# CloudEngineHub/FairyGen

Measured on AMD Instinct MI355X. Metric: decoded frames/sec (sec/clip in config), Wan2.2-TI2V-5B 704x1280x121 @ 5 steps, higher is better.
Workload: dtype bf16

## Files before the change

### fairygen_amd/csrc/attention.hip

```cpp
#include "common.h"
#include <math.h>
#include <queue>
#include <type_traits>
#include <vector>

#include "attn_w4_asm.inc"
#include "attn_w4p_asm.inc"
#ifndef FG_ATTN_W4
#define FG_ATTN_W4 1
#endif

namespace {

constexpr int kD = 128;
constexpr int kBN = 64;
constexpr int kTileBytes = kBN * kD * 2;
constexpr float kDeferLog2 = 6.0f;

typedef __attribute__((address_space(3))) s16x4 lds_s16x4;

__device__ __forceinline__ int k_lds_off(int row, int chunk) { return row * 256 + ((chunk ^ (row & 15)) << 4); }
__device__ __forceinline__ int v_lds_off(int row, int chunk) {
    return 2048 * (row >> 3) + 512 * (chunk >> 2) + 64 * (row & 7) + 16 * ((chunk & 3) ^ ((row >> 2) & 3));
}
// ... 531 lines not shown
    std::priority_queue<double, std::vector<double>, std::greater<double>> free_at;
    for (int i = 0; i < cus; ++i) free_at.push((double)(full + (i < rem ? 1 : 0)));
    double last = (double)(full + (rem ? 1 : 0));
    for (int64_t i = 0; i < n_pieces; ++i) {
        const double t = free_at.top() + piece_cost;
        free_at.pop();
        free_at.push(t);
        last = t > last ? t : last;
    }
    return last;
}

static SplitChoice choose_split_uncached(int B, int64_t Nq, int64_t Nkv, int H, int cus, int64_t ws_limit) {
    const int64_t nqb = (Nq + kBM - 1) / kBM, bh = (int64_t)B * H;
    const int nt = (int)((Nkv + kBN - 1) / kBN);
    const int64_t per_piece = (int64_t)kBM * kD * 4 + (int64_t)kBM * 2 * 4;
    SplitChoice best{0, 1, 0, simulate_makespan(bh * nqb, 0, 0.0, cus)};
    const double base = best.makespan;
    const int s_list[] = {2, 3, 4, 5, 6, 8, 12, 16};
    for (int mode = 0; mode < 2; ++mode) {
        const int64_t R = mode == 0 ? 1 : nqb;
        if (mode == 0 && nqb < 2) continue;
        if (mode == 1 && bh * nqb > 4 * (int64_t)cus) continue;
        for (int S : s_list) {
            if (S * 8 > nt) break;
            const int64_t pieces = bh * R * S;
            const int64_t ws = pieces * per_piece;
            if (ws > ws_limit) continue;
            const double cost = 1.0 / S + 3.0 / nt + 0.004;
            const double ms = simulate_makespan(bh * (nqb - R), pieces, cost, cus);
            if (ms < best.makespan) best = SplitChoice{(int)R, S, ws, ms};
        }
    }
    if (best.makespan > 0.98 * base) best = SplitChoice{0, 1, 0, base};
    return best;
}

static SplitChoice choose_split(int B, int64_t Nq, int64_t Nkv, int H, int cus, int64_t ws_limit) {
    struct Key { int B, H, cus; int64_t Nq, Nkv, ws; SplitChoice val; };
    static thread_local Key memo[8];
    static thread_local int next = 0, filled = 0;
    for (int i = 0; i < filled; ++i) {
        const Key& e = memo[i];
        if (e.B == B && e.H == H && e.cus == cus && e.Nq == Nq && e.Nkv == Nkv && e.ws == ws_limit) return e.val;
    }
    const SplitChoice val = choose_split_uncached(B, Nq, Nkv, H, cus, ws_limit);
    memo[next] = Key{B, H, cus, Nq, Nkv, ws_limit, val};
    next = (next + 1) % 8;
    if (filled < 8) ++filled;
    return val;
}

static int device_cus() {
    static thread_local int cached_dev = -1, cached_cus = 256;
    int dev = 0;
    if (hipGetDevice(&dev) != hipSuccess) return 256;
    if (dev != cached_dev) {
        int n = 0;
        if (hipDeviceGetAttribute(&n, hipDeviceAttributeMultiprocessorCount, dev) == hipSuccess && n > 0) cached_cus = n;
        cached_dev = dev;
    }
    return cached_cus * (256 / kBM);
}

}

extern "C" int64_t fg_attn_workspace_bytes(int B, int64_t Nq, int64_t Nkv, int H) {
    if (B <= 0 || Nq <= 0 || Nkv <= 0 || H <= 0) return 0;
    return choose_split(B, Nq, Nkv, H, device_cus(), (int64_t)1 << 40).ws_bytes;
}

extern "C" int fg_attn_split_choice(int B, int64_t Nq, int64_t Nkv, int H, int64_t workspace_bytes, int* R, int* S) {
    FG_CHECK_ARG(B > 0 && Nq > 0 && Nkv > 0 && H > 0 && R && S, "fg_attn_split_choice: bad arguments");
    const SplitChoice sc = choose_split(B, Nq, Nkv, H, device_cus(), workspace_bytes);
    *R = sc.R;
    *S = sc.S;
    return FG_OK;
}

extern "C" int fg_attn_fwd_bf16(const void* q, int64_t ldq, const void* k, int64_t ldk, const void* v, int64_t ldv,
                                void* out, int B, int64_t Nq, int64_t Nkv, int H, int D, float scale, void* workspace,
                                int64_t workspace_bytes, fg_stream_t stream) {
    FG_CHECK_ARG(q && k && v && out, "fg_attn_fwd_bf16: null pointer");
    FG_CHECK_ARG(D == kD, "fg_attn_fwd_bf16: only head_dim 128 is supported (got %d)", D);
    FG_CHECK_ARG(B > 0 && H > 0 && Nq > 0 && Nkv > 0, "fg_attn_fwd_bf16: B, H, Nq, Nkv must be positive");
    FG_CHECK_ARG(scale > 0.f, "fg_attn_fwd_bf16: scale must be positive");
    const int64_t hd = (int64_t)H * D;
    FG_CHECK_ARG(ldq >= hd && ldk >= hd && ldv >= hd && ldq % 8 == 0 && ldk % 8 == 0 && ldv % 8 == 0,
                 "fg_attn_fwd_bf16: leading dimensions must be >= H*D and multiples of 8");
    FG_CHECK_ARG(FG_ALIGNED16(q) && FG_ALIGNED16(k) && FG_ALIGNED16(v) && FG_ALIGNED16(out) && FG_ALIGNED16(workspace),
                 "fg_attn_fwd_bf16: pointers must be 16-byte aligned");
    FG_CHECK_ARG(workspace_bytes >= 0 && (workspace != nullptr || workspace_bytes == 0), "fg_attn_fwd_bf16: bad workspace");
    const int64_t nqb = (Nq + kBM - 1) / kBM;
    FG_CHECK_ARG((Nkv + 6 * kBN) * ldk * 2 < (1ll << 32) && (Nkv + 6 * kBN) * ldv * 2 < (1ll << 32),
                 "fg_attn_fwd_bf16: K/V of one batch element must span < 4 GiB (32-bit buffer offsets)");
    FG_CHECK_ARG(Nq * ldq * 2 < (1ll << 32) && Nq * hd * 2 < (1ll << 32),
                 "fg_attn_fwd_bf16: Q / O of one batch element must span < 4 GiB (32-bit buffer offsets)");
    const SplitChoice sc = choose_split(B, Nq, Nkv, H, device_cus(), workspace_bytes);
    AttnParams P;
    P.q = (const bf16*)q; P.k = (const bf16*)k; P.v = (const bf16*)v; P.out = (bf16*)out;
    P.ldq = ldq; P.ldk = ldk; P.ldv = ldv; P.Nq = Nq; P.Nkv = Nkv; P.H = H;
    P.nqb = (int)nqb; P.R = sc.R; P.S = sc.S; P.nfull = (int)(nqb - sc.R);
    const int64_t total_direct = (int64_t)B * H * P.nfull, pieces = (int64_t)B * H * sc.R * sc.S;
    FG_CHECK_ARG(total_direct + pieces < (1ll << 30), "fg_attn_fwd_bf16: grid too large");
    P.total_direct = (int)total_direct;
    P.scale_log2e = scale * 1.4426950408889634f;
    P.o_part = (float*)workspace;
    P.ml_part = (float*)workspace + pieces * kBM * kD;
#if FG_ATTN_VARIANT == 4
    hipLaunchKernelGGL((attn_fwd_kernel<4, 1>), dim3((unsigned)(total_direct + pieces)), dim3(256), 0, (hipStream_t)stream, P);
#else
#if FG_ATTN_W4
    static const bool use_w4 = [] { const char* e = getenv("FAIRYGEN_ATTN_W4"); return e ? atoi(e) != 0 : true; }();
    if (Nkv > 1024 && use_w4) {
        static const hipError_t attr0 = hipFuncSetAttribute(reinterpret_cast<const void*>(attn_fwd_w4_kernel<false>),
// ... 27 lines not shown
```

### fairygen_amd/csrc/common.h

```cpp
#pragma once
#include <hip/hip_runtime.h>
#include <stdint.h>
#include <stdio.h>
#include "../../include/fairygen_hip.h"

typedef __bf16 bf16;
typedef __attribute__((ext_vector_type(8))) __bf16 bf16x8;
typedef __attribute__((ext_vector_type(4))) __bf16 bf16x4;
typedef __attribute__((ext_vector_type(2))) __bf16 bf16x2;
typedef __attribute__((ext_vector_type(16))) float f32x16;
typedef __attribute__((ext_vector_type(4))) float f32x4;
typedef __attribute__((ext_vector_type(4))) short s16x4;
typedef __attribute__((ext_vector_type(4))) uint32_t u32x4;
typedef __attribute__((ext_vector_type(2))) uint32_t u32x2;

#define FG_WAVE 64

void fg_set_error(const char* fmt, ...);

#define FG_CHECK_ARG(cond, ...)                                  \
    do {                                                         \
        if (!(cond)) {                                           \
            fg_set_error(__VA_ARGS__);                           \
            return FG_EINVAL;                                    \
        }                                                        \
    } while (0)

#define FG_ALIGNED16(p) ((((uintptr_t)(p)) & 15) == 0)

static inline int fg_launch_status(const char* what) {
    hipError_t e = hipGetLastError();
    if (e != hipSuccess) {
        fg_set_error("%s: launch failed: %s", what, hipGetErrorString(e));
        return FG_ELAUNCH;
    }
    return FG_OK;
}

__device__ __forceinline__ float rbf(float x) { return (float)(bf16)x; }

__device__ __forceinline__ float silu_f(float x) { return x / (1.0f + __expf(-x)); }
__device__ __forceinline__ float gelu_tanh_f(float x) {
    const float kBeta = 0.7978845608028654f, kKappa = 0.044715f;
    const float u = kBeta * (x + kKappa * x * x * x);
    const float e = __expf(2.0f * fminf(u, 15.0f));
    const float t = 1.0f - 2.0f / (1.0f + e);
    return 0.5f * x * (1.0f + t);
}

__device__ __forceinline__ float gelu_tanh_epilogue(float y) {
    const float c1 = (float)(-2.0 * 0.7978845608028654 * 1.4426950408889634), c2 = (float)(-2.0 * 0.7978845608028654 * 1.4426950408889634 * 0.044715);
    const float arg = __builtin_fmaf(y * y, c2, c1) * y;
    return y * __builtin_amdgcn_rcpf(__builtin_amdgcn_exp2f(arg) + 1.0f);
}

__device__ __forceinline__ float wave_sum(float v) {
#pragma unroll
    for (int o = 32; o > 0; o >>= 1) v += __shfl_xor(v, o, 64);
    return v;
}
__device__ __forceinline__ float wave_max(float v) {
#pragma unroll
    for (int o = 32; o > 0; o >>= 1) v = fmaxf(v, __shfl_xor(v, o, 64));
    return v;
}

template <int NW>
__device__ __forceinline__ float block_sum(float v, float* red) {
    v = wave_sum(v);
    if (NW == 1) return v;
    const int w = threadIdx.x >> 6;
    __syncthreads();
    if ((threadIdx.x & 63) == 0) red[w] = v;
    __syncthreads();
    float t = 0.f;
#pragma unroll
    for (int i = 0; i < NW; ++i) t += red[i];
    return t;
}
```

### fairygen_amd/csrc/dit_elementwise.hip

```cpp
#include "common.h"

#ifndef FG_ROW_MIN_WAVES
#define FG_ROW_MIN_WAVES 4
#endif
#define FG_ROW_BOUNDS __launch_bounds__(256, FG_ROW_MIN_WAVES)

namespace {

constexpr int kMaxVec = 8;
constexpr int kRowsPerBlock = 4;

struct Row {
    float v[kMaxVec][8];
};

__device__ __forceinline__ void load_row(const bf16* p, int C, int lane, Row& r) {
    const int nvec = C >> 3;
#pragma unroll
    for (int i = 0; i < kMaxVec; ++i) {
        const int vi = lane + i * 64;
        if (vi < nvec) {
            bf16x8 t = *reinterpret_cast<const bf16x8*>(p + (int64_t)vi * 8);
#pragma unroll
            for (int j = 0; j < 8; ++j) r.v[i][j] = (float)t[j];
        } else {
#pragma unroll
            for (int j = 0; j < 8; ++j) r.v[i][j] = 0.f;
        }
    }
}

__device__ __forceinline__ bf16x8 ld8(const bf16* p) { return *reinterpret_cast<const bf16x8*>(p); }
__device__ __forceinline__ void st8(bf16* p, const float* f) {
    bf16x8 t;
#pragma unroll
    for (int j = 0; j < 8; ++j) t[j] = (bf16)f[j];
    *reinterpret_cast<bf16x8*>(p) = t;
}

__device__ __forceinline__ void row_moments(const Row& r, int C, int lane, float eps, float& mean, float& rstd) {
    const int nvec = C >> 3;
    float s = 0.f;
#pragma unroll
    for (int i = 0; i < kMaxVec; ++i)
#pragma unroll
        for (int j = 0; j < 8; ++j) s += r.v[i][j];
    mean = wave_sum(s) / (float)C;
    float q = 0.f;
#pragma unroll
    for (int i = 0; i < kMaxVec; ++i) {
        if (lane + i * 64 < nvec) {
#pragma unroll
            for (int j = 0; j < 8; ++j) {
                const float d = r.v[i][j] - mean;
                q += d * d;
            }
        }
    }
// ... 238 lines not shown
                        const double a = (double)o[2 * j], b = (double)o[2 * j + 1];
                        const double c = cp[j], sn = sp[j];
                        o[2 * j] = (float)(bf16)(a * c - b * sn);
                        o[2 * j + 1] = (float)(bf16)(a * sn + b * c);
                    }
                }
            }
            const int col = vi * 8, g = PLAIN ? 0 : col / group_cols;
            st8(out + g * out_group_stride + row * out_ld + (col - g * group_cols), o);
        }
    }
}

__global__ __launch_bounds__(256) void copy_groups_kernel(const bf16* __restrict__ src, int64_t sgs, int64_t sld,
                                                          bf16* __restrict__ dst, int64_t dgs, int64_t dld, int groups,
                                                          int64_t rows, int vec_per_row) {
    const int64_t total = (int64_t)groups * rows * vec_per_row;
    for (int64_t i = (int64_t)blockIdx.x * blockDim.x + threadIdx.x; i < total; i += (int64_t)gridDim.x * blockDim.x) {
        const int64_t rg = i / vec_per_row;
        const int v = (int)(i - rg * vec_per_row);
        const int64_t r = rg / groups;
        const int g = (int)(rg - r * groups);
        *reinterpret_cast<u32x4*>(dst + g * dgs + r * dld + v * 8) =
            *reinterpret_cast<const u32x4*>(src + g * sgs + r * sld + v * 8);
    }
}


template <int KIND>
__global__ __launch_bounds__(256) void act_kernel(const bf16* __restrict__ x, bf16* __restrict__ out, int64_t nvec) {
    for (int64_t i = (int64_t)blockIdx.x * blockDim.x + threadIdx.x; i < nvec; i += (int64_t)gridDim.x * blockDim.x) {
        const bf16x8 v = ld8(x + i * 8);
        float o[8];
#pragma unroll
        for (int j = 0; j < 8; ++j) o[j] = KIND == 0 ? silu_f((float)v[j]) : gelu_tanh_f((float)v[j]);
        st8(out + i * 8, o);
    }
}

__global__ __launch_bounds__(256) void cfg_euler_kernel(const bf16* __restrict__ lat, const bf16* __restrict__ posi,
                                                        const bf16* __restrict__ nega, bf16* __restrict__ out,
                                                        int64_t n, float cfg, float dsigma) {
    for (int64_t i = (int64_t)blockIdx.x * blockDim.x + threadIdx.x; i < n; i += (int64_t)gridDim.x * blockDim.x) {
        const float p = (float)posi[i];
        float pred = p;
        if (nega != nullptr) {
            const float ng = (float)nega[i];
            pred = rbf(ng + rbf(cfg * rbf(p - ng)));
        }
        out[i] = (bf16)((float)lat[i] + rbf(pred * dsigma));
    }
}

inline int check_rows(const char* fn, int64_t rows, int C, int64_t mod_rows, int64_t first_rows) {
    FG_CHECK_ARG(rows >= 0 && C > 0 && (C % 8) == 0 && C <= kMaxVec * 512, "%s: need C %% 8 == 0 and C <= %d (got rows=%lld C=%d)",
                 fn, kMaxVec * 512, (long long)rows, C);
    FG_CHECK_ARG(mod_rows == 1 || mod_rows == 2 || mod_rows == rows, "%s: mod_rows must be 1, 2 or rows (got %lld)", fn,
                 (long long)mod_rows);
    FG_CHECK_ARG(first_rows >= 0 && first_rows <= rows, "%s: first_rows out of range", fn);
    return FG_OK;
}

inline dim3 row_grid(int64_t rows) { return dim3((unsigned)((rows + kRowsPerBlock - 1) / kRowsPerBlock)); }

}

extern "C" {

int fg_ln_modulate_bf16(const void* x, const void* shift, const void* scale, void* out, int64_t rows, int C, float eps,
                        int64_t mod_rows, int64_t first_rows, int64_t mod_ld, fg_stream_t stream) {
    if (int e = check_rows("fg_ln_modulate_bf16", rows, C, mod_rows, first_rows)) return e;
    FG_CHECK_ARG(x && shift && scale && out, "fg_ln_modulate_bf16: null pointer");
    FG_CHECK_ARG(FG_ALIGNED16(x) && FG_ALIGNED16(shift) && FG_ALIGNED16(scale) && FG_ALIGNED16(out) && mod_ld % 8 == 0,
                 "fg_ln_modulate_bf16: pointers / mod_ld must be 16-byte aligned");
    if (rows == 0) return FG_OK;
    hipLaunchKernelGGL(ln_modulate_kernel, row_grid(rows), dim3(256), 0, (hipStream_t)stream, (const bf16*)x,
                       (const bf16*)shift, (const bf16*)scale, (bf16*)out, rows, C, eps, mod_rows, first_rows, mod_ld);
    return fg_launch_status("fg_ln_modulate_bf16");
}

int fg_ln_modulate_fp8_bf16(const void* x, const void* shift, const void* scale, void* out_fp8, float* out_scale, int64_t rows, int C,
                            float eps, int64_t mod_rows, int64_t first_rows, int64_t mod_ld, float fp8_max, fg_stream_t stream) {
    if (int e = check_rows("fg_ln_modulate_fp8_bf16", rows, C, mod_rows, first_rows)) return e;
    FG_CHECK_ARG(x && shift && scale && out_fp8 && out_scale, "fg_ln_modulate_fp8_bf16: null pointer");
    FG_CHECK_ARG(FG_ALIGNED16(x) && FG_ALIGNED16(shift) && FG_ALIGNED16(scale) && (((uintptr_t)out_fp8) & 7) == 0 && mod_ld % 8 == 0 &&
                     fp8_max > 0.f,
                 "fg_ln_modulate_fp8_bf16: pointers / mod_ld must be 16-byte aligned (out_fp8: 8), fp8_max positive");
    if (rows == 0) return FG_OK;
    hipLaunchKernelGGL(ln_modulate_fp8_kernel, row_grid(rows), dim3(256), 0, (hipStream_t)stream, (const bf16*)x, (const bf16*)shift,
                       (const bf16*)scale, (uint8_t*)out_fp8, out_scale, rows, C, eps, mod_rows, first_rows, mod_ld, fp8_max);
    return fg_launch_status("fg_ln_modulate_fp8_bf16");
}

int fg_ln_modulate_dual_bf16(const void* x, const void* shift, const void* scale, void* out, void* out_fp8, float* out_scale,
                             int64_t rows, int C, float eps, int64_t mod_rows, int64_t first_rows, int64_t mod_ld, float fp8_max,
                             fg_stream_t stream) {
    if (int e = check_rows("fg_ln_modulate_dual_bf16", rows, C, mod_rows, first_rows)) return e;
    FG_CHECK_ARG(x && shift && scale && out && out_fp8 && out_scale, "fg_ln_modulate_dual_bf16: null pointer");
    FG_CHECK_ARG(FG_ALIGNED16(x) && FG_ALIGNED16(shift) && FG_ALIGNED16(scale) && FG_ALIGNED16(out) && (((uintptr_t)out_fp8) & 7) == 0 &&
                     mod_ld % 8 == 0 && fp8_max > 0.f,
                 "fg_ln_modulate_dual_bf16: pointers / mod_ld must be 16-byte aligned (out_fp8: 8), fp8_max positive");
    if (rows == 0) return FG_OK;
    hipLaunchKernelGGL(ln_dual_kernel<0>, row_grid(rows), dim3(256), 0, (hipStream_t)stream, (const bf16*)x, (const bf16*)shift,
                       (const bf16*)scale, (bf16*)out, (uint8_t*)out_fp8, out_scale, rows, C, eps, mod_rows, first_rows, mod_ld, fp8_max);
    return fg_launch_status("fg_ln_modulate_dual_bf16");
}

int fg_ln_affine_dual_bf16(const void* x, const void* w, const void* b, void* out, void* out_fp8, float* out_scale, int64_t rows, int C,
                           float eps, float fp8_max, fg_stream_t stream) {
    if (int e = check_rows("fg_ln_affine_dual_bf16", rows, C, 1, 0)) return e;
    FG_CHECK_ARG(x && w && b && out && out_fp8 && out_scale, "fg_ln_affine_dual_bf16: null pointer");
    FG_CHECK_ARG(FG_ALIGNED16(x) && FG_ALIGNED16(w) && FG_ALIGNED16(b) && FG_ALIGNED16(out) && (((uintptr_t)out_fp8) & 7) == 0 &&
                     fp8_max > 0.f,
                 "fg_ln_affine_dual_bf16: pointers must be 16-byte aligned (out_fp8: 8), fp8_max positive");
    if (rows == 0) return FG_OK;
    hipLaunchKernelGGL(ln_dual_kernel<1>, row_grid(rows), dim3(256), 0, (hipStream_t)stream, (const bf16*)x, (const bf16*)w,
                       (const bf16*)b, (bf16*)out, (uint8_t*)out_fp8, out_scale, rows, C, eps, (int64_t)1, (int64_t)0, (int64_t)0, fp8_max);
    return fg_launch_status("fg_ln_affine_dual_bf16");
}

int fg_residual_ln_fp8_bf16(const void* x, const void* y, const void* gate, void* x_out, const void* p0, const void* p1,
                            void* norm_fp8, float* norm_scale, int mode, int64_t rows, int C, float eps, int64_t mod_rows,
                            int64_t first_rows, int64_t mod_ld, float fp8_max, fg_stream_t stream) {
    FG_CHECK_ARG(mode == 0 || mode == 1, "fg_residual_ln_fp8_bf16: mode must be 0 (modulate) or 1 (affine)");
    const bool need_mod = gate != nullptr || mode == 0;
    if (int e = check_rows("fg_residual_ln_fp8_bf16", rows, C, need_mod ? mod_rows : 1, need_mod ? first_rows : 0)) return e;
    FG_CHECK_ARG(x && y && x_out && p0 && p1 && norm_fp8 && norm_scale, "fg_residual_ln_fp8_bf16: null pointer");
    FG_CHECK_ARG(FG_ALIGNED16(x) && FG_ALIGNED16(y) && FG_ALIGNED16(gate) && FG_ALIGNED16(x_out) && FG_ALIGNED16(p0) &&
                     FG_ALIGNED16(p1) && (((uintptr_t)norm_fp8) & 7) == 0 && mod_ld % 8 == 0 && fp8_max > 0.f,
                 "fg_residual_ln_fp8_bf16: pointers / mod_ld must be 16-byte aligned (norm_fp8: 8), fp8_max positive");
    if (rows == 0) return FG_OK;
    if (!need_mod) { mod_rows = 1; first_rows = 0; }
    if (mode == 0)
        hipLaunchKernelGGL(residual_kernel<0>, row_grid(rows), dim3(256), 0, (hipStream_t)stream, (const bf16*)x,
                           (const bf16*)y, (const bf16*)gate, (bf16*)x_out, (const bf16*)p0, (const bf16*)p1,
                           (bf16*)nullptr, rows, C, eps, mod_rows, first_rows, mod_ld, (uint8_t*)norm_fp8, norm_scale, fp8_max);
    else
        hipLaunchKernelGGL(residual_kernel<1>, row_grid(rows), dim3(256), 0, (hipStream_t)stream, (const bf16*)x,
                           (const bf16*)y, (const bf16*)gate, (bf16*)x_out, (const bf16*)p0, (const bf16*)p1,
                           (bf16*)nullptr, rows, C, eps, mod_rows, first_rows, mod_ld, (uint8_t*)norm_fp8, norm_scale, fp8_max);
    return fg_launch_status("fg_residual_ln_fp8_bf16");
}

int fg_ln_affine_bf16(const void* x, const void* w, const void* b, void* out, int64_t rows, int C, float eps,
                      fg_stream_t stream) {
    if (int e = check_rows("fg_ln_affine_bf16", rows, C, 1, 0)) return e;
    FG_CHECK_ARG(x && w && b && out, "fg_ln_affine_bf16: null pointer");
    FG_CHECK_ARG(FG_ALIGNED16(x) && FG_ALIGNED16(w) && FG_ALIGNED16(b) && FG_ALIGNED16(out),
                 "fg_ln_affine_bf16: pointers must be 16-byte aligned");
    if (rows == 0) return FG_OK;
    hipLaunchKernelGGL(ln_affine_kernel, row_grid(rows), dim3(256), 0, (hipStream_t)stream, (const bf16*)x, (const bf16*)w,
                       (const bf16*)b, (bf16*)out, rows, C, eps);
    return fg_launch_status("fg_ln_affine_bf16");
}

int fg_gate_residual_bf16(const void* x, const void* y, const void* gate, void* out, int64_t rows, int C, int64_t mod_rows,
                          int64_t first_rows, int64_t mod_ld, fg_stream_t stream) {
    if (int e = check_rows("fg_gate_residual_bf16", rows, C, gate ? mod_rows : 1, gate ? first_rows : 0)) return e;
    FG_CHECK_ARG(x && y && out, "fg_gate_residual_bf16: null pointer");
    FG_CHECK_ARG(FG_ALIGNED16(x) && FG_ALIGNED16(y) && FG_ALIGNED16(gate) && FG_ALIGNED16(out) && mod_ld % 8 == 0,
                 "fg_gate_residual_bf16: pointers / mod_ld must be 16-byte aligned");
    if (rows == 0) return FG_OK;
    hipLaunchKernelGGL(residual_kernel<-1>, row_grid(rows), dim3(256), 0, (hipStream_t)stream, (const bf16*)x,
                       (const bf16*)y, (const bf16*)gate, (bf16*)out, (const bf16*)nullptr, (const bf16*)nullptr,
                       (bf16*)nullptr, rows, C, 0.f, gate ? mod_rows : 1, gate ? first_rows : 0, mod_ld);
    return fg_launch_status("fg_gate_residual_bf16");
}

int fg_residual_ln_bf16(const void* x, const void* y, const void* gate, void* x_out, const void* p0, const void* p1,
                        void* norm_out, int mode, int64_t rows, int C, float eps, int64_t mod_rows, int64_t first_rows,
                        int64_t mod_ld, fg_stream_t stream) {
    FG_CHECK_ARG(mode == 0 || mode == 1, "fg_residual_ln_bf16: mode must be 0 (modulate) or 1 (affine)");
    const bool need_mod = gate != nullptr || mode == 0;
    if (int e = check_rows("fg_residual_ln_bf16", rows, C, need_mod ? mod_rows : 1, need_mod ? first_rows : 0)) return e;
    FG_CHECK_ARG(x && y && x_out && p0 && p1 && norm_out, "fg_residual_ln_bf16: null pointer");
    FG_CHECK_ARG(FG_ALIGNED16(x) && FG_ALIGNED16(y) && FG_ALIGNED16(gate) && FG_ALIGNED16(x_out) && FG_ALIGNED16(p0) &&
                     FG_ALIGNED16(p1) && FG_ALIGNED16(norm_out) && mod_ld % 8 == 0,
                 "fg_residual_ln_bf16: pointers / mod_ld must be 16-byte aligned");
    if (rows == 0) return FG_OK;
    if (!need_mod) { mod_rows = 1; first_rows = 0; }
    if (mode == 0)
        hipLaunchKernelGGL(residual_kernel<0>, row_grid(rows), dim3(256), 0, (hipStream_t)stream, (const bf16*)x,
                           (const bf16*)y, (const bf16*)gate, (bf16*)x_out, (const bf16*)p0, (const bf16*)p1,
                           (bf16*)norm_out, rows, C, eps, mod_rows, first_rows, mod_ld);
    else
        hipLaunchKernelGGL(residual_kernel<1>, row_grid(rows), dim3(256), 0, (hipStream_t)stream, (const bf16*)x,
                           (const bf16*)y, (const bf16*)gate, (bf16*)x_out, (const bf16*)p0, (const bf16*)p1,
                           (bf16*)norm_out, rows, C, eps, mod_rows, first_rows, mod_ld);
    return fg_launch_status("fg_residual_ln_bf16");
}

int fg_rmsnorm_rope_bf16(const void* x, int64_t ldx, const void* weight, const void* cos_tab, const void* sin_tab,
                         int table_f32, void* out, int64_t rows, int C, int num_heads, float eps, fg_stream_t stream) {
    if (int e = check_rows("fg_rmsnorm_rope_bf16", rows, C, 1, 0)) return e;
    FG_CHECK_ARG(x && weight && out, "fg_rmsnorm_rope_bf16: null pointer");
    FG_CHECK_ARG(table_f32 ? (cos_tab != nullptr && sin_tab == nullptr) : ((cos_tab == nullptr) == (sin_tab == nullptr)),
                 "fg_rmsnorm_rope_bf16: fp64 mode takes both tables or neither, fp32 mode ONE interleaved table in cos_tab");
    FG_CHECK_ARG(num_heads > 0 && C % num_heads == 0 && (C / num_heads) % 8 == 0,
                 "fg_rmsnorm_rope_bf16: head_dim must be a multiple of 8");
    FG_CHECK_ARG(ldx >= C && ldx % 8 == 0 && FG_ALIGNED16(x) && FG_ALIGNED16(weight) && FG_ALIGNED16(out) &&
                     FG_ALIGNED16(cos_tab) && FG_ALIGNED16(sin_tab),
                 "fg_rmsnorm_rope_bf16: pointers / ldx must be 16-byte aligned");
    if (rows == 0) return FG_OK;
    const int hd = C / num_heads;
    const bool plain = (hd & (hd - 1)) == 0;
#define FG_ROPE_LAUNCH(TAB, PL)                                                                                                  \
    hipLaunchKernelGGL((rmsnorm_rope_kernel<TAB, PL>), row_grid(rows), dim3(256), 0, (hipStream_t)stream, (const bf16*)x, ldx,    \
                       (const bf16*)weight, cos_tab, sin_tab, (bf16*)out, rows, C, hd, eps, C, (int64_t)0, (int64_t)C)
    if (table_f32) { if (plain) FG_ROPE_LAUNCH(true, true); else FG_ROPE_LAUNCH(true, false); }
    else { if (plain) FG_ROPE_LAUNCH(false, true); else FG_ROPE_LAUNCH(false, false); }
#undef FG_ROPE_LAUNCH
    return fg_launch_status("fg_rmsnorm_rope_bf16");
}

int fg_rmsnorm_rope_grouped_bf16(const void* x, int64_t ldx, const void* weight, const void* cos_tab,
                                 const void* sin_tab, int table_f32, void* out, int64_t rows, int C, int num_heads, float eps,
                                 int group_cols, int64_t out_group_stride, int64_t out_ld, fg_stream_t stream) {
    if (int e = check_rows("fg_rmsnorm_rope_grouped_bf16", rows, C, 1, 0)) return e;
    FG_CHECK_ARG(x && weight && out, "fg_rmsnorm_rope_grouped_bf16: null pointer");
    FG_CHECK_ARG(table_f32 ? (cos_tab != nullptr && sin_tab == nullptr) : ((cos_tab == nullptr) == (sin_tab == nullptr)),
                 "fg_rmsnorm_rope_grouped_bf16: fp64 mode takes both tables or neither, fp32 mode ONE interleaved table in cos_tab");
    FG_CHECK_ARG(num_heads > 0 && C % num_heads == 0 && (C / num_heads) % 8 == 0,
                 "fg_rmsnorm_rope_grouped_bf16: head_dim must be a multiple of 8");
    FG_CHECK_ARG(group_cols > 0 && group_cols % 8 == 0 && C % group_cols == 0 && out_ld >= group_cols && out_ld % 8 == 0 &&
                     out_group_stride % 8 == 0 && out_group_stride >= 0,
                 "fg_rmsnorm_rope_grouped_bf16: group_cols must divide C; group_cols, out_ld, out_group_stride multiples of 8");
    FG_CHECK_ARG(ldx >= C && ldx % 8 == 0 && FG_ALIGNED16(x) && FG_ALIGNED16(weight) && FG_ALIGNED16(out) &&
                     FG_ALIGNED16(cos_tab) && FG_ALIGNED16(sin_tab),
                 "fg_rmsnorm_rope_grouped_bf16: pointers / ldx must be 16-byte aligned");
    if (rows == 0) return FG_OK;
    if (table_f32)
        hipLaunchKernelGGL((rmsnorm_rope_kernel<true, false>), row_grid(rows), dim3(256), 0, (hipStream_t)stream, (const bf16*)x, ldx,
                           (const bf16*)weight, cos_tab, sin_tab, (bf16*)out, rows, C, C / num_heads, eps, group_cols,
                           out_group_stride, out_ld);
    else
        hipLaunchKernelGGL((rmsnorm_rope_kernel<false, false>), row_grid(rows), dim3(256), 0, (hipStream_t)stream, (const bf16*)x, ldx,
                           (const bf16*)weight, cos_tab, sin_tab, (bf16*)out, rows, C, C / num_heads, eps, group_cols,
                           out_group_stride, out_ld);
    return fg_launch_status("fg_rmsnorm_rope_grouped_bf16");
}

int fg_copy_groups_bf16(const void* src, int64_t src_group_stride, int64_t src_ld, void* dst, int64_t dst_group_stride,
                        int64_t dst_ld, int groups, int64_t rows, int cols, fg_stream_t stream) {
    FG_CHECK_ARG(src && dst, "fg_copy_groups_bf16: null pointer");
    FG_CHECK_ARG(groups > 0 && rows >= 0 && cols > 0 && cols % 8 == 0, "fg_copy_groups_bf16: cols must be a positive multiple of 8");
    FG_CHECK_ARG(src_group_stride % 8 == 0 && src_ld % 8 == 0 && dst_group_stride % 8 == 0 && dst_ld % 8 == 0 &&
                     src_ld >= cols && dst_ld >= cols && FG_ALIGNED16(src) && FG_ALIGNED16(dst),
                 "fg_copy_groups_bf16: strides must be multiples of 8 elements, rows at least cols wide, pointers 16-byte aligned");
    if (rows == 0) return FG_OK;
    const int64_t total = (int64_t)groups * rows * (cols / 8);
    const unsigned grid = (unsigned)((total + 255) / 256 < 16384 ? (total + 255) / 256 : 16384);
    hipLaunchKernelGGL(copy_groups_kernel, dim3(grid), dim3(256), 0, (hipStream_t)stream, (const bf16*)src, src_group_stride,
                       src_ld, (bf16*)dst, dst_group_stride, dst_ld, groups, rows, cols / 8);
    return fg_launch_status("fg_copy_groups_bf16");
}

int fg_act_bf16(const void* x, void* out, int64_t n, int kind, fg_stream_t stream) {
    FG_CHECK_ARG(x && out && n >= 0 && n % 8 == 0, "fg_act_bf16: n must be a multiple of 8");
// ... 24 lines not shown
```

### fairygen_amd/hip.py

```python
import ctypes
import os

import torch

_LIB_PATH = os.environ.get("FAIRYGEN_HIP_LIB") or os.path.join(os.path.dirname(os.path.abspath(__file__)), "libfairygen_hip.so")
_lib = None

ABI_VERSION = 7

_i64, _i32, _f32, _vp = ctypes.c_int64, ctypes.c_int, ctypes.c_float, ctypes.c_void_p

_SIGNATURES = {
    "fg_ln_modulate_bf16": [_vp, _vp, _vp, _vp, _i64, _i32, _f32, _i64, _i64, _i64, _vp],
    "fg_ln_affine_bf16": [_vp, _vp, _vp, _vp, _i64, _i32, _f32, _vp],
    "fg_ln_modulate_fp8_bf16": [_vp, _vp, _vp, _vp, _vp, _i64, _i32, _f32, _i64, _i64, _i64, _f32, _vp],
    "fg_residual_ln_fp8_bf16": [_vp, _vp, _vp, _vp, _vp, _vp, _vp, _vp, _i32, _i64, _i32, _f32, _i64, _i64, _i64, _f32, _vp],
    "fg_ln_modulate_dual_bf16": [_vp, _vp, _vp, _vp, _vp, _vp, _i64, _i32, _f32, _i64, _i64, _i64, _f32, _vp],
    "fg_ln_affine_dual_bf16": [_vp, _vp, _vp, _vp, _vp, _vp, _i64, _i32, _f32, _f32, _vp],
    "fg_gate_residual_bf16": [_vp, _vp, _vp, _vp, _i64, _i32, _i64, _i64, _i64, _vp],
    "fg_residual_ln_bf16": [_vp, _vp, _vp, _vp, _vp, _vp, _vp, _i32, _i64, _i32, _f32, _i64, _i64, _i64, _vp],
    "fg_rmsnorm_rope_bf16": [_vp, _i64, _vp, _vp, _vp, _i32, _vp, _i64, _i32, _i32, _f32, _vp],
    "fg_rmsnorm_rope_grouped_bf16": [_vp, _i64, _vp, _vp, _vp, _i32, _vp, _i64, _i32, _i32, _f32, _i32, _i64, _i64, _vp],
    "fg_copy_groups_bf16": [_vp, _i64, _i64, _vp, _i64, _i64, _i32, _i64, _i32, _vp],
    "fg_fp8_quant_rows_bf16": [_vp, _i64, _vp, _vp, _vp, _i64, _i32, _i32, _f32, _vp],
    "fg_act_bf16": [_vp, _vp, _i64, _i32, _vp],
    "fg_gemm_epilogue_bf16": [_vp, _i64, _vp, _vp, _vp, _i64, _i64, _i64, _i64, _i32, _vp, _i64, _i64, _i64, _vp, _vp],
    "fg_gemm_fp8_bf16": [_vp, _i64, _vp, _vp, _vp, _vp, _i64, _i64, _i64, _i64, _i32, _vp, _i64, _i64, _i64, _vp, _vp],
    "fg_gemm_sched_reset": [_vp, _vp],
    "fg_gemm_epilogue_bf16_s": [_vp, _i64, _vp, _vp, _vp, _i64, _i64, _i64, _i64, _i32, _vp, _i64, _i64, _i64, _vp, _vp, _i32, _vp],
    "fg_gemm_fp8_bf16_s": [_vp, _i64, _vp, _vp, _vp, _vp, _i64, _i64, _i64, _i64, _i32, _vp, _i64, _i64, _i64, _vp, _vp, _i32, _vp],
    "fg_lora_apply_bf16": [_vp, _i64, _vp, _vp, _vp, _i64, _i64, _i64, _i64, _i64, _i64, _i32, _vp, _i64, _i64, _i64, _vp],
    "fg_attn_fwd_bf16": [_vp, _i64, _vp, _i64, _vp, _i64, _vp, _i32, _i64, _i64, _i32, _i32, _f32, _vp, _i64, _vp],
    "fg_cfg_euler_bf16": [_vp, _vp, _vp, _vp, _i64, _f32, _f32, _vp],
    "fg_vae_rmsnorm_silu_bf16": [_vp, _vp, _vp, _i64, _i32, _i32, _vp],
    "fg_conv_pack_weight_bf16": [_vp, _vp, _i32, _i32, _i32, _i32, _i32, _vp],
    "fg_conv3d_cl_bf16": [_vp, _vp, _vp, _vp, _vp, _i32, _i32, _i32, _i32, _i32, _i32, _i32, _i32, _i32, _vp],
    "fg_dupup3d_add_bf16": [_vp, _vp, _vp, _i32, _i32, _i32, _i32, _i32, _i32, _i32, _i32, _vp],
    "fg_softmax_rows_f32_bf16": [_vp, _vp, _i64, _i64, _f32, _vp],
    "fg_vae_latent_to_cl_bf16": [_vp, _vp, _vp, _vp, _i32, _i32, _i32, _i32, _vp],
    "fg_vae_unpatchify_bf16": [_vp, _vp, _i32, _i32, _i32, _i32, _i32, _i32, _vp],
    "fg_vae_tile_accumulate_bf16": [_vp, _vp, _vp, _i32, _i32, _i32, _i32, _i32, _i32, _i32, _i32, _i32, _i32, _i32, _vp],
    "fg_vae_tile_finalize_bf16": [_vp, _vp, _i32, _i32, _i32, _i32, _i32, _vp],
    "fg_vae_patchify_bf16": [_vp, _vp, _i32, _i32, _i32, _vp],
    "fg_avgdown3d_add_bf16": [_vp, _vp, _vp, _i32, _i32, _i32, _i32, _i32, _i32, _i32, _vp],
    "fg_vae_latent_from_cl_bf16": [_vp, _vp, _vp, _vp, _i32, _i32, _i32, _i32, _i32, _vp],
    "fg_video_to_uint8": [_vp, _vp, _i32, _i32, _i32, _vp],
    "fg_softmax_bias_bf16": [_vp, _vp, _vp, _vp, _i64, _i64, _vp],
    "fg_gated_gelu_bf16": [_vp, _vp, _vp, _i64, _vp],
}
_LOAD_TIME_SIGNATURES = {
    "fg_lora_fuse_bf16": [_vp, _i64, _vp, _i64, _vp, _i64, _vp, _vp, _i64, _i64, _i64, _f32, _vp],
}
EXPORTED_SYMBOLS = sorted(list(_SIGNATURES) + list(_LOAD_TIME_SIGNATURES) + ["fg_version", "fg_last_error", "fg_conv_packed_bytes", "fg_attn_workspace_bytes", "fg_attn_split_choice",
                                                   "fg_conv_tile_choice", "fg_gemm_workspace_bytes", "fg_gemm_debug_grid", "fg_gemm_sched_bytes"])


class HipLibraryError(RuntimeError):
    pass


def library_path():
# ... 642 lines not shown
```

Baseline: 15.92.

## Add persistent row kernels with register prefetch for LayerNorm, residual, and RoPE

Adds grid-stride persistent variants of the LayerNorm-modulate, LayerNorm-affine, gated-residual, residual+LN, and RMSNorm+RoPE kernels. The grid is sized to CUs times the minimum waves per SIMD. Each wave prefetches the next row into registers while it normalizes the current one, and reloads modulation parameters only when the row's class changes. The goal is to hide global-load latency and avoid reloading the shift/scale/gate vectors for every row. The cost is higher register pressure (launch bounds of 2 waves), lower occupancy, and extra template instantiations. The CU-count lookup moves into a shared helper.

```diff
diff --git a/fairygen_amd/csrc/attention.hip b/fairygen_amd/csrc/attention.hip
--- a/fairygen_amd/csrc/attention.hip
+++ b/fairygen_amd/csrc/attention.hip
@@ -607,15 +607,7 @@
 }
 
 static int device_cus() {
-    static thread_local int cached_dev = -1, cached_cus = 256;
-    int dev = 0;
-    if (hipGetDevice(&dev) != hipSuccess) return 256;
-    if (dev != cached_dev) {
-        int n = 0;
-        if (hipDeviceGetAttribute(&n, hipDeviceAttributeMultiprocessorCount, dev) == hipSuccess && n > 0) cached_cus = n;
-        cached_dev = dev;
-    }
-    return cached_cus * (256 / kBM);
+    return fg_device_cus() * (256 / kBM);
 }
 
 }
diff --git a/fairygen_amd/csrc/common.h b/fairygen_amd/csrc/common.h
--- a/fairygen_amd/csrc/common.h
+++ b/fairygen_amd/csrc/common.h
@@ -35,6 +35,18 @@
         return FG_ELAUNCH;
     }
     return FG_OK;
+}
+
+static inline int fg_device_cus() {
+    static thread_local int cached_dev = -1, cached_cus = 256;
+    int dev = 0;
+    if (hipGetDevice(&dev) != hipSuccess) return 256;
+    if (dev != cached_dev) {
+        int n = 0;
+        if (hipDeviceGetAttribute(&n, hipDeviceAttributeMultiprocessorCount, dev) == hipSuccess && n > 0) cached_cus = n;
+        cached_dev = dev;
+    }
+    return cached_cus;
 }
 
 __device__ __forceinline__ float rbf(float x) { return (float)(bf16)x; }
diff --git a/fairygen_amd/csrc/dit_elementwise.hip b/fairygen_amd/csrc/dit_elementwise.hip
--- a/fairygen_amd/csrc/dit_elementwise.hip
+++ b/fairygen_amd/csrc/dit_elementwise.hip
@@ -4,6 +4,11 @@
 #define FG_ROW_MIN_WAVES 4
 #endif
 #define FG_ROW_BOUNDS __launch_bounds__(256, FG_ROW_MIN_WAVES)
+
+#ifndef FG_PROW_MIN_WAVES
+#define FG_PROW_MIN_WAVES 2
+#endif
+#define FG_PROW_BOUNDS __launch_bounds__(256, FG_PROW_MIN_WAVES)
 
 namespace {
 
@@ -348,6 +353,283 @@
     }
 }
 
+constexpr int kPersistRowsPerCU = 16;
+
+template <int NV> struct RowN { float v[NV][8]; };
+template <int NV> struct PackN { bf16x8 v[NV]; };
+
+template <int NV, bool PK> struct ParamN;
+template <int NV> struct ParamN<NV, false> {
+    float v[NV][8];
+    __device__ __forceinline__ float get(int i, int j) const { return v[i][j]; }
+    __device__ __forceinline__ void set(int i, int j, float f) { v[i][j] = f; }
+};
+template <int NV> struct ParamN<NV, true> {
+    bf16x8 v[NV];
+    __device__ __forceinline__ float get(int i, int j) const { return (float)v[i][j]; }
+    __device__ __forceinline__ void set(int i, int j, float f) { v[i][j] = (bf16)f; }
+};
+
+template <int NV>
+__device__ __forceinline__ void load_pack(const bf16* p, int nvec, int lane, PackN<NV>& t) {
+#pragma unroll
+    for (int i = 0; i < NV; ++i) {
+        const int vi = lane + i * 64;
+        if (vi < nvec) {
+            t.v[i] = ld8(p + (int64_t)vi * 8);
+        } else {
+#pragma unroll
+            for (int j = 0; j < 8; ++j) t.v[i][j] = (bf16)0.f;
+        }
+    }
+}
+
+template <int NV>
+__device__ __forceinline__ void unpack_row(const PackN<NV>& t, RowN<NV>& r) {
+#pragma unroll
+    for (int i = 0; i < NV; ++i)
+#pragma unroll
+        for (int j = 0; j < 8; ++j) r.v[i][j] = (float)t.v[i][j];
+}
+
+template <int KIND, int NV, bool PK>
+__device__ __forceinline__ void load_param(const bf16* p, int nvec, int lane, ParamN<NV, PK>& a) {
+#pragma unroll
+    for (int i = 0; i < NV; ++i) {
+        const int vi = lane + i * 64;
+        if (vi < nvec) {
+            const bf16x8 t = ld8(p + (int64_t)vi * 8);
+#pragma unroll
+            for (int j = 0; j < 8; ++j) a.set(i, j, KIND == 1 ? rbf(1.0f + (float)t[j]) : (float)t[j]);
+        } else {
+#pragma unroll
+            for (int j = 0; j < 8; ++j) a.set(i, j, 0.f);
+        }
+    }
+}
+
+template <int NV>
+__device__ __forceinline__ void row_moments_n(const RowN<NV>& r, int C, int lane, float eps, float& mean, float& rstd) {
+    const int nvec = C >> 3;
+    float s = 0.f;
+#pragma unroll
+    for (int i = 0; i < NV; ++i)
+#pragma unroll
+        for (int j = 0; j < 8; ++j) s += r.v[i][j];
+    mean = wave_sum(s) / (float)C;
+    float q = 0.f;
+#pragma unroll
+    for (int i = 0; i < NV; ++i) {
+        if (lane + i * 64 < nvec) {
+#pragma unroll
+            for (int j = 0; j < 8; ++j) {
+                const float d = r.v[i][j] - mean;
+                q += d * d;
+            }
+        }
+    }
+    const float var = wave_sum(q) / (float)C;
+    rstd = 1.0f / sqrtf(var + eps);
+}
+
+template <int MODE, int NV, bool PK>
+__device__ __forceinline__ void norm_store_reg(const RowN<NV>& r, int C, int lane, float eps, const ParamN<NV, PK>& a,
+                                               const ParamN<NV, PK>& b, bf16* out) {
+    const int nvec = C >> 3;
+    float mean, rstd;
+    row_moments_n(r, C, lane, eps, mean, rstd);
+#pragma unroll
+    for (int i = 0; i < NV; ++i) {
+        const int vi = lane + i * 64;
+        if (vi < nvec) {
+            float o[8];
+#pragma unroll
+            for (int j = 0; j < 8; ++j) {
+                const float n = (r.v[i][j] - mean) * rstd;
+                if (MODE == 0) {
+                    const float y = rbf(n);
+                    const float s1 = b.get(i, j);
+                    o[j] = rbf(y * s1) + a.get(i, j);
+                } else {
+                    o[j] = n * a.get(i, j) + b.get(i, j);
+                }
+            }
+            st8(out + (int64_t)vi * 8, o);
+        }
+    }
+}
+
+__device__ __forceinline__ int64_t persist_first_row() {
+    return (int64_t)blockIdx.x * kRowsPerBlock + __builtin_amdgcn_readfirstlane((int)(threadIdx.x >> 6));
+}
+__device__ __forceinline__ int64_t persist_stride() { return (int64_t)gridDim.x * kRowsPerBlock; }
+
+template <int MODE, int NV>
+__global__ FG_PROW_BOUNDS void ln_persist_kernel(const bf16* __restrict__ x, const bf16* __restrict__ p0, const bf16* __restrict__ p1,
+                                                 bf16* __restrict__ out, int64_t rows, int C, float eps, int64_t mod_rows,
+                                                 int64_t first_rows, int64_t mod_ld) {
+    const int lane = threadIdx.x & 63, nvec = C >> 3;
+    const int64_t stride = persist_stride();
+    int64_t row = persist_first_row();
+    if (row >= rows) return;
+    PackN<NV> nxt;
+    load_pack(x + row * C, nvec, lane, nxt);
+    int64_t cls = MODE == 0 ? mod_row(row, mod_rows, first_rows) : 0;
+    ParamN<NV, false> a, b;
+    load_param<0>(p0 + cls * mod_ld, nvec, lane, a);
+    load_param<MODE == 0 ? 1 : 0>(p1 + cls * mod_ld, nvec, lane, b);
+    for (; row < rows; row += stride) {
+        RowN<NV> r;
+        unpack_row(nxt, r);
+        if (row + stride < rows) load_pack(x + (row + stride) * C, nvec, lane, nxt);
+        const int64_t m = MODE == 0 ? mod_row(row, mod_rows, first_rows) : 0;
+        if (m != cls) {
+            cls = m;
+            load_param<0>(p0 + cls * mod_ld, nvec, lane, a);
+            load_param<MODE == 0 ? 1 : 0>(p1 + cls * mod_ld, nvec, lane, b);
+        }
+        norm_store_reg<MODE>(r, C, lane, eps, a, b, out + row * C);
+    }
+}
+
+template <int MODE, int NV>
+__global__ FG_PROW_BOUNDS void residual_persist_kernel(const bf16* __restrict__ x, const bf16* __restrict__ y,
+                                                       const bf16* __restrict__ gate, bf16* __restrict__ x_out,
+                                                       const bf16* __restrict__ p0, const bf16* __restrict__ p1,
+                                                       bf16* __restrict__ norm_out, int64_t rows, int C, float eps, int64_t mod_rows,
+                                                       int64_t first_rows, int64_t mod_ld) {
+    const int lane = threadIdx.x & 63, nvec = C >> 3;
+    const int64_t stride = persist_stride();
+    int64_t row = persist_first_row();
+    if (row >= rows) return;
+    PackN<NV> nx, ny;
+    load_pack(x + row * C, nvec, lane, nx);
+    load_pack(y + row * C, nvec, lane, ny);
+    int64_t cls = -1;
+    ParamN<NV, true> g, a, b;
+    for (; row < rows; row += stride) {
+        const PackN<NV> cx = nx, cy = ny;
+        if (row + stride < rows) {
+            load_pack(x + (row + stride) * C, nvec, lane, nx);
+            load_pack(y + (row + stride) * C, nvec, lane, ny);
+        }
+        const int64_t m = mod_row(row, mod_rows, first_rows);
+        if (m != cls) {
+            cls = m;
+            if (gate != nullptr) load_param<0>(gate + cls * mod_ld, nvec, lane, g);
+            if (MODE == 0) {
+                load_param<0>(p0 + cls * mod_ld, nvec, lane, a);
+                load_param<1>(p1 + cls * mod_ld, nvec, lane, b);
+            }
+            if (MODE == 1) {
+                load_param<0>(p0, nvec, lane, a);
+                load_param<0>(p1, nvec, lane, b);
+            }
+        }
+        RowN<NV> r;
+#pragma unroll
+        for (int i = 0; i < NV; ++i) {
+            const int vi = lane + i * 64;
+            if (vi < nvec) {
+                if (gate != nullptr) {
+#pragma unroll
+                    for (int j = 0; j < 8; ++j) r.v[i][j] = rbf((float)cx.v[i][j] + rbf(g.get(i, j) * (float)cy.v[i][j]));
+                } else {
+#pragma unroll
+                    for (int j = 0; j < 8; ++j) r.v[i][j] = rbf((float)cx.v[i][j] + (float)cy.v[i][j]);
+                }
+                st8(x_out + row * C + (int64_t)vi * 8, r.v[i]);
+            } else {
+#pragma unroll
+                for (int j = 0; j < 8; ++j) r.v[i][j] = 0.f;
+            }
+        }
+        if (MODE >= 0) norm_store_reg<(MODE < 0 ? 0 : MODE)>(r, C, lane, eps, a, b, norm_out + row * C);
+    }
+}
+
+template <bool F32TAB, bool PLAIN, int NV>
+__global__ FG_PROW_BOUNDS void rmsnorm_rope_persist_kernel(const bf16* __restrict__ x, int64_t ldx, const bf16* __restrict__ w,
+                                                           const void* __restrict__ ctv, const void* __restrict__ stv,
+                                                           bf16* __restrict__ out, int64_t rows, int C, int head_dim, float eps) {
+    const int lane = threadIdx.x & 63, nvec = C >> 3;
+    const int64_t stride = persist_stride();
+    int64_t row = persist_first_row();
+    if (row >= rows) return;
+    const int half = head_dim >> 1;
+    const bool hoist = F32TAB && ctv != nullptr && (512 % head_dim) == 0;
+    const int d_lane = PLAIN ? ((lane * 8) & (head_dim - 1)) : ((lane * 8) % head_dim);
+    PackN<NV> nxt;
+    load_pack(x + row * ldx, nvec, lane, nxt);
+    f32x4 n0 = {0.f, 0.f, 0.f, 0.f}, n1 = {0.f, 0.f, 0.f, 0.f};
+    if (hoist) {
+        const f32x4* tp = reinterpret_cast<const f32x4*>(static_cast<const float*>(ctv) + (row * half + (d_lane >> 1)) * 2);
+        n0 = tp[0];
+        n1 = tp[1];
+    }
+    ParamN<NV, false> wv;
+    load_param<0>(w, nvec, lane, wv);
+    for (; row < rows; row += stride) {
+        RowN<NV> r;
+        unpack_row(nxt, r);
+        const f32x4 h0 = n0, h1 = n1;
+        if (row + stride < rows) {
+            load_pack(x + (row + stride) * ldx, nvec, lane, nxt);
+            if (hoist) {
+                const f32x4* tp =
+                    reinterpret_cast<const f32x4*>(static_cast<const float*>(ctv) + ((row + stride) * half + (d_lane >> 1)) * 2);
+                n0 = tp[0];
+                n1 = tp[1];
+            }
+        }
+        float q = 0.f;
+#pragma unroll
+        for (int i = 0; i < NV; ++i)
+#pragma unroll
+            for (int j = 0; j < 8; ++j) q += r.v[i][j] * r.v[i][j];
+        const float ms = wave_sum(q) / (float)C;
+        const float rinv = 1.0f / sqrtf(ms + eps);
+#pragma unroll
+        for (int i = 0; i < NV; ++i) {
+            const int vi = lane + i * 64;
+            if (vi < nvec) {
+                float o[8];
+#pragma unroll
+                for (int j = 0; j < 8; ++j) o[j] = rbf(rbf(r.v[i][j] * rinv) * wv.get(i, j));
+                if (ctv != nullptr) {
+                    const int d0 = PLAIN ? ((vi * 8) & (head_dim - 1)) : ((vi * 8) % head_dim);
+                    if (F32TAB) {
+                        f32x4 t0 = h0, t1 = h1;
+                        if (!hoist) {
+                            const f32x4* tp = reinterpret_cast<const f32x4*>(static_cast<const float*>(ctv) + (row * half + (d0 >> 1)) * 2);
+                            t0 = tp[0];
+                            t1 = tp[1];
+                        }
+                        const float cs[8] = {t0[0], t0[1], t0[2], t0[3], t1[0], t1[1], t1[2], t1[3]};
+#pragma unroll
+                        for (int j = 0; j < 4; ++j) {
+                            const float a = o[2 * j], b = o[2 * j + 1], c = cs[2 * j], sn = cs[2 * j + 1];
+                            o[2 * j] = rbf(__builtin_fmaf(a, c, -(b * sn)));
+                            o[2 * j + 1] = rbf(__builtin_fmaf(a, sn, b * c));
+                        }
+                    } else {
+                        const double* cp = static_cast<const double*>(ctv) + row * half + (d0 >> 1);
+                        const double* sp = static_cast<const double*>(stv) + row * half + (d0 >> 1);
+#pragma unroll
+                        for (int j = 0; j < 4; ++j) {
+                            const double a = (double)o[2 * j], b = (double)o[2 * j + 1];
+                            const double c = cp[j], sn = sp[j];
+                            o[2 * j] = (float)(bf16)(a * c - b * sn);
+                            o[2 * j + 1] = (float)(bf16)(a * sn + b * c);
+                        }
+                    }
+                }
+                st8(out + row * C + (int64_t)vi * 8, o);
+            }
+        }
+    }
+}
+
 inline int check_rows(const char* fn, int64_t rows, int C, int64_t mod_rows, int64_t first_rows) {
     FG_CHECK_ARG(rows >= 0 && C > 0 && (C % 8) == 0 && C <= kMaxVec * 512, "%s: need C %% 8 == 0 and C <= %d (got rows=%lld C=%d)",
                  fn, kMaxVec * 512, (long long)rows, C);
@@ -359,6 +641,12 @@
 
 inline dim3 row_grid(int64_t rows) { return dim3((unsigned)((rows + kRowsPerBlock - 1) / kRowsPerBlock)); }
 
+inline bool use_persist(int64_t rows, int64_t mod_rows) {
+    return rows > (int64_t)kPersistRowsPerCU * fg_device_cus() && (mod_rows == 1 || mod_rows == 2);
+}
+inline dim3 persist_grid() { return dim3((unsigned)(fg_device_cus() * FG_PROW_MIN_WAVES)); }
+#define FG_PERSIST_NV(C, LAUNCH) do { if ((C) <= 6 * 512) { LAUNCH(6); } else { LAUNCH(8); } } while (0)
+
 }
 
 extern "C" {
@@ -370,6 +658,13 @@
     FG_CHECK_ARG(FG_ALIGNED16(x) && FG_ALIGNED16(shift) && FG_ALIGNED16(scale) && FG_ALIGNED16(out) && mod_ld % 8 == 0,
                  "fg_ln_modulate_bf16: pointers / mod_ld must be 16-byte aligned");
     if (rows == 0) return FG_OK;
+    if (use_persist(rows, mod_rows)) {
+#define FG_L(NV) hipLaunchKernelGGL((ln_persist_kernel<0, NV>), persist_grid(), dim3(256), 0, (hipStream_t)stream, (const bf16*)x,  \
+                                    (const bf16*)shift, (const bf16*)scale, (bf16*)out, rows, C, eps, mod_rows, first_rows, mod_ld)
+        FG_PERSIST_NV(C, FG_L);
+#undef FG_L
+        return fg_launch_status("fg_ln_modulate_bf16");
+    }
     hipLaunchKernelGGL(ln_modulate_kernel, row_grid(rows), dim3(256), 0, (hipStream_t)stream, (const bf16*)x,
                        (const bf16*)shift, (const bf16*)scale, (bf16*)out, rows, C, eps, mod_rows, first_rows, mod_ld);
     return fg_launch_status("fg_ln_modulate_bf16");
@@ -445,6 +740,13 @@
     FG_CHECK_ARG(FG_ALIGNED16(x) && FG_ALIGNED16(w) && FG_ALIGNED16(b) && FG_ALIGNED16(out),
                  "fg_ln_affine_bf16: pointers must be 16-byte aligned");
     if (rows == 0) return FG_OK;
+    if (use_persist(rows, 1)) {
+#define FG_L(NV) hipLaunchKernelGGL((ln_persist_kernel<1, NV>), persist_grid(), dim3(256), 0, (hipStream_t)stream, (const bf16*)x,  \
+                                    (const bf16*)w, (const bf16*)b, (bf16*)out, rows, C, eps, (int64_t)1, (int64_t)0, (int64_t)0)
+        FG_PERSIST_NV(C, FG_L);
+#undef FG_L
+        return fg_launch_status("fg_ln_affine_bf16");
+    }
     hipLaunchKernelGGL(ln_affine_kernel, row_grid(rows), dim3(256), 0, (hipStream_t)stream, (const bf16*)x, (const bf16*)w,
                        (const bf16*)b, (bf16*)out, rows, C, eps);
     return fg_launch_status("fg_ln_affine_bf16");
@@ -457,6 +759,15 @@
     FG_CHECK_ARG(FG_ALIGNED16(x) && FG_ALIGNED16(y) && FG_ALIGNED16(gate) && FG_ALIGNED16(out) && mod_ld % 8 == 0,
                  "fg_gate_residual_bf16: pointers / mod_ld must be 16-byte aligned");
     if (rows == 0) return FG_OK;
+    if (use_persist(rows, gate ? mod_rows : 1)) {
+#define FG_L(NV) hipLaunchKernelGGL((residual_persist_kernel<-1, NV>), persist_grid(), dim3(256), 0, (hipStream_t)stream,           \
+                                    (const bf16*)x, (const bf16*)y, (const bf16*)gate, (bf16*)out, (const bf16*)nullptr,             \
+                                    (const bf16*)nullptr, (bf16*)nullptr, rows, C, 0.f, gate ? mod_rows : 1, gate ? first_rows : 0,  \
+                                    mod_ld)
+        FG_PERSIST_NV(C, FG_L);
+#undef FG_L
+        return fg_launch_status("fg_gate_residual_bf16");
+    }
     hipLaunchKernelGGL(residual_kernel<-1>, row_grid(rows), dim3(256), 0, (hipStream_t)stream, (const bf16*)x,
                        (const bf16*)y, (const bf16*)gate, (bf16*)out, (const bf16*)nullptr, (const bf16*)nullptr,
                        (bf16*)nullptr, rows, C, 0.f, gate ? mod_rows : 1, gate ? first_rows : 0, mod_ld);
@@ -475,6 +786,22 @@
                  "fg_residual_ln_bf16: pointers / mod_ld must be 16-byte aligned");
     if (rows == 0) return FG_OK;
     if (!need_mod) { mod_rows = 1; first_rows = 0; }
+    if (use_persist(rows, mod_rows)) {
+#define FG_L(NV)                                                                                                                    \
+    do {                                                                                                                            \
+        if (mode == 0)                                                                                                              \
+            hipLaunchKernelGGL((residual_persist_kernel<0, NV>), persist_grid(), dim3(256), 0, (hipStream_t)stream, (const bf16*)x, \
+                               (const bf16*)y, (const bf16*)gate, (bf16*)x_out, (const bf16*)p0, (const bf16*)p1, (bf16*)norm_out,  \
+                               rows, C, eps, mod_rows, first_rows, mod_ld);                                                         \
+        else                                                                                                                        \
+            hipLaunchKernelGGL((residual_persist_kernel<1, NV>), persist_grid(), dim3(256), 0, (hipStream_t)stream, (const bf16*)x, \
+                               (const bf16*)y, (const bf16*)gate, (bf16*)x_out, (const bf16*)p0, (const bf16*)p1, (bf16*)norm_out,  \
+                               rows, C, eps, mod_rows, first_rows, mod_ld);                                                         \
+    } while (0)
+        FG_PERSIST_NV(C, FG_L);
+#undef FG_L
+        return fg_launch_status("fg_residual_ln_bf16");
+    }
     if (mode == 0)
         hipLaunchKernelGGL(residual_kernel<0>, row_grid(rows), dim3(256), 0, (hipStream_t)stream, (const bf16*)x,
                            (const bf16*)y, (const bf16*)gate, (bf16*)x_out, (const bf16*)p0, (const bf16*)p1,
@@ -500,6 +827,20 @@
     if (rows == 0) return FG_OK;
     const int hd = C / num_heads;
     const bool plain = (hd & (hd - 1)) == 0;
+    if (use_persist(rows, 1)) {
+#define FG_ROPE_P(TAB, PL, NV)                                                                                                      \
+    hipLaunchKernelGGL((rmsnorm_rope_persist_kernel<TAB, PL, NV>), persist_grid(), dim3(256), 0, (hipStream_t)stream, (const bf16*)x, \
+                       ldx, (const bf16*)weight, cos_tab, sin_tab, (bf16*)out, rows, C, hd, eps)
+#define FG_L(NV)                                                                                                                    \
+    do {                                                                                                                            \
+        if (table_f32) { if (plain) FG_ROPE_P(true, true, NV); else FG_ROPE_P(true, false, NV); }                                   \
+        else { if (plain) FG_ROPE_P(false, true, NV); else FG_ROPE_P(false, false, NV); }                                           \
+    } while (0)
+        FG_PERSIST_NV(C, FG_L);
+#undef FG_L
+#undef FG_ROPE_P
+        return fg_launch_status("fg_rmsnorm_rope_bf16");
+    }
 #define FG_ROPE_LAUNCH(TAB, PL)                                                                                                  \
     hipLaunchKernelGGL((rmsnorm_rope_kernel<TAB, PL>), row_grid(rows), dim3(256), 0, (hipStream_t)stream, (const bf16*)x, ldx,    \
                        (const bf16*)weight, cos_tab, sin_tab, (bf16*)out, rows, C, hd, eps, C, (int64_t)0, (int64_t)C)
diff --git a/fairygen_amd/hip.py b/fairygen_amd/hip.py
--- a/fairygen_amd/hip.py
+++ b/fairygen_amd/hip.py
@@ -7,6 +7,8 @@
 _lib = None
 
 ABI_VERSION = 7
+
+PERSISTENT_ROWS_PER_CU = 16
 
 _i64, _i32, _f32, _vp = ctypes.c_int64, ctypes.c_int, ctypes.c_float, ctypes.c_void_p
 
```

Measured after the change: 16.00, median of 5. No clear change (+0.5%).
